# C0ldstudy/PointSecGuard

Hardware: AMD Instinct MI355X
Metric: attacked rooms/sec (4096 pts, 40 PGD iters) (higher is better)
Workload: dtype f32; 1 GPU; NB non-targeted PGD (eps=0.05, alpha=2/255, 40 iters) on PointNet++ SSG sem_seg, batch=8 rooms x 4096 pts x 9 ch per GPU (BASELINE configs[1]); steps_coalesced_per_launch_max=8, device_batch_rooms=64, launches_in_flight_per_gpu=3, weights=tests/golden/pn2_weights.npz (fitted fixture)

## Files before the change

pointsecguard_amd/csrc/psg_api.hip:

```cpp
#include <mutex>
#include <atomic>
#include <stdarg.h>
#include <stdlib.h>
#include <string.h>
#include <unordered_set>

#include "psg_common.h"

namespace {
thread_local char g_err[512] = "";
}

namespace psg {
struct EnvSwitch { const char *name; char kind; };
static const EnvSwitch kEnvSwitches[] = {
    {"PSG_TRACE_SYNC", 'd'},       {"PSG_GCN_KNN_STATS", 'd'},   {"PSG_KNN_XCD_ORDER", 'p'},  {"PSG_KNN_FINE_CUT_KK", 'p'},  {"PSG_KNN_SAMPLE2_KK", 'p'},  {"PSG_KNN_F32_SAMPLED_KK", 'p'},
    {"PSG_FP1_WAVE", 'p'},         {"PSG_RLA_NO_FUSE16", 'p'},   {"PSG_RLA_ATOMICS", 'p'},    {"PSG_RLA_NO_SPLIT", 'p'},
    {"PSG_RLA_NO_GRAPH", 'p'},     {"PSG_GEMM_SMALL_BELOW", 'p'}, {"PSG_GCN_KNN", 'p'},        {"PSG_GCN_KNN_BF_MAXD", 'p'},
    {"PSG_GCN_PQ_FUSION", 'p'},    {"PSG_GCN_NO_GRAPH", 'p'},    {"PSG_GCN_EDGE_BWD", 'p'},   {"PSG_BALL_QUERY", 'p'},
    {"PSG_PN2_SPLIT", 'p'},          {"PSG_RLA_NO_DIRECT", 'p'},   {"PSG_NU_NO_GRAPH", 'p'},      {"PSG_PN2_GRAPH", 'p'},
    {"PSG_PN2_FPSPLIT", 'p'},        {"PSG_FPS_CFG", 'p'},         {"PSG_PN2_L1T_COLOUR", 'p'},
    {"PSG_PN2_PGD_FUSE", 'p'},       {"PSG_PN2_POOLT_SPARSE", 'p'}, {"PSG_PN2_PW_SIZED", 'p'},
    {"PSG_PN2_BALL_TABLE", 'p'},     {"PSG_PN2_PACK", 'p'},          {"PSG_PN2_PACK_BWD", 'p'},
    {"PSG_PN2_POOLT_ORDER", 'p'},
#ifdef PSG_DIAG_BUILD
    {"PSG_DIAG", 'r'},
#endif
};

hipError_t copy_sync(void *dst, const void *src, size_t bytes, hipMemcpyKind kind)
{
    if (bytes == 0) return hipSuccess;
    hipStream_t st = nullptr;
    hipError_t e = hipStreamCreateWithFlags(&st, hipStreamNonBlocking);
    if (e != hipSuccess) return e;
    e = hipMemcpyAsync(dst, src, bytes, kind, st);
    if (e == hipSuccess) e = hipStreamSynchronize(st);
    (void)hipStreamDestroy(st);
    return e;
}

static std::atomic<uint64_t> g_generation{0};
uint64_t next_generation() { return ++g_generation; }

static std::atomic<long long> g_capture[4];
void capture_note(CaptureCounters *own, int tried, int failed, int replays, int eager)
{
    if (own) { own->tried += tried; own->failed += failed; own->replays += replays; own->eager += eager; }
    g_capture[0] += tried; g_capture[1] += failed; g_capture[2] += replays; g_capture[3] += eager;
}

bool GraphSlot::capture(hipStream_t st, const std::function<int()> &body)
{
    bool ok = false;
    if (hipStreamBeginCapture(st, hipStreamCaptureModeThreadLocal) == hipSuccess) {
        const int crc = body();
        hipGraph_t graph = nullptr;
        const hipError_t e = hipStreamEndCapture(st, &graph);
        ok = crc == PSG_OK && e == hipSuccess && graph && hipGraphInstantiate(&exec, graph, nullptr, nullptr, 0) == hipSuccess;
        if (!ok) exec = nullptr;
        if (graph) (void)hipGraphDestroy(graph);
    }
    (void)hipGetLastError();
    capture_failed = !ok;
    capture_note(&cap, 1, ok ? 0 : 1, 0, 0);
    return ok;
}

hipError_t GraphSlot::forget(hipStream_t st)
{
    if (exec) {
        const hipError_t e = hipStreamSynchronize(st);
        if (e != hipSuccess) return e;
        destroy();
    }
    capture_failed = false;
    return hipSuccess;
}

hipError_t GraphSlot::replay(hipStream_t st, int n)
{
    capture_note(&cap, 0, 0, n, 0);
    for (int i = 0; i < n; ++i) {
        const hipError_t e = hipGraphLaunch(exec, st);
        if (e != hipSuccess) return e;
    }
    return hipSuccess;
}

void GraphSlot::destroy()
{
    if (exec) (void)hipGraphExecDestroy(exec);
    exec = nullptr;
}

hipError_t memset_sync(void *dst, int value, size_t bytes)
{
    if (bytes == 0) return hipSuccess;
    hipStream_t st = nullptr;
    hipError_t e = hipStreamCreateWithFlags(&st, hipStreamNonBlocking);
    if (e != hipSuccess) return e;
    e = hipMemsetAsync(dst, value, bytes, st);
    if (e == hipSuccess) e = hipStreamSynchronize(st);
    (void)hipStreamDestroy(st);
    return e;
}

const char *env_str(const char *name)
{
    bool known = false;
    for (const EnvSwitch &e : kEnvSwitches) known = known || strcmp(e.name, name) == 0;
    if (!known) fprintf(stderr, "[psg] environment switch %s is read but not registered in psg_api.hip\n", name);
    return getenv(name);
}

int env_int(const char *name, int dflt)
{
    const char *v = env_str(name);
    return v ? atoi(v) : dflt;
}

bool trace_sync_enabled()
{
    static const bool on = env_int("PSG_TRACE_SYNC", 0) != 0;
    return on;
}

void trace_sync_point(const char *site)
{
    static unsigned long n = 0;
    const char *base = strrchr(site, '/');
    fprintf(stderr, "[psg trace] launch %lu at %s issued\n", ++n, base ? base + 1 : site);
    fflush(stderr);
    hipError_t e = hipDeviceSynchronize();
    fprintf(stderr, "[psg trace] launch %lu done (%s)\n", n, hipGetErrorString(e));
    fflush(stderr);
}

hipError_t allow_big_lds(const void *kern)
{
    static std::mutex mu;
    static std::unordered_set<const void *> done;
    std::lock_guard<std::mutex> lock(mu);
    if (done.count(kern)) return hipSuccess;
    hipFuncAttributes fa;
    hipError_t e = hipFuncGetAttributes(&fa, kern);
    if (e == hipSuccess) e = hipFuncSetAttribute(kern, hipFuncAttributeMaxDynamicSharedMemorySize, 160 * 1024 - (int)fa.sharedSizeBytes);
    if (e == hipSuccess) done.insert(kern);
    if (trace_sync_enabled()) fprintf(stderr, "[psg trace] LDS opt-in %zu (%s)\n", done.size(), hipGetErrorString(e));
    return e;
}

void set_error(const char *fmt, ...)
{
    va_list ap;
    va_start(ap, fmt);
    vsnprintf(g_err, sizeof(g_err), fmt, ap);
    va_end(ap);
}
}

extern "C" const char *psg_last_error(void) { return g_err; }

extern "C" int psg_env_switches(char *buf, int cap)
{
    PSG_REQUIRE(buf && cap > 0, "psg_env_switches: null / empty buffer");
    std::string out;
    int n = 0;
    for (const psg::EnvSwitch &e : psg::kEnvSwitches) {
        const char *v = getenv(e.name);
        if (!v) continue;
        out += std::string(e.name) + "=" + v + ":" + e.kind + ";";
        ++n;
    }
    PSG_REQUIRE((int)out.size() < cap, "psg_env_switches: buffer of %d bytes is too small (%d needed)", cap, (int)out.size() + 1);
    memcpy(buf, out.c_str(), out.size() + 1);
    return n;
}

extern "C" int psg_diag_build(void)
{
#ifdef PSG_DIAG_BUILD
    return 1;
#else
    return 0;
#endif
}

extern "C" int psg_capture_stats(long long *out4)
{
    PSG_REQUIRE(out4, "psg_capture_stats: null out pointer");
    for (int i = 0; i < 4; ++i) out4[i] = psg::g_capture[i].load();
    return PSG_OK;
}

extern "C" const char *psg_version(void) { return "libpsg 0.1 (gfx950, fp32 MFMA)"; }

extern "C" int psg_ctx_create(int device, psg_ctx **out)
{
    PSG_REQUIRE(out, "psg_ctx_create: null out pointer");
    int n = 0;
    PSG_CHECK_HIP(hipGetDeviceCount(&n));
    PSG_REQUIRE(device >= 0 && device < n, "psg_ctx_create: device %d not present (%d devices)", device, n);
    hipDeviceProp_t prop;
    PSG_CHECK_HIP(hipGetDeviceProperties(&prop, device));
    if (std::string(prop.gcnArchName).rfind("gfx950", 0) != 0) {
        psg::set_error("psg_ctx_create: device %d is %s; libpsg is built for gfx950 (MI355X) only", device,
                       prop.gcnArchName);
        return PSG_ERR_ARG;
    }
    PSG_CHECK_HIP(hipSetDevice(device));
    psg_ctx *c = new psg_ctx();
    c->device = device;
    c->num_cu = prop.multiProcessorCount;
    *out = c;
    return PSG_OK;
}

extern "C" int psg_ctx_destroy(psg_ctx *ctx)
{
    delete ctx;
    return PSG_OK;
}
```

pointsecguard_amd/csrc/psg_geometry.hip:

```cpp
#include "psg_common.h"
#include "psg_sqdist.cuh"

namespace {

using psg::sqdist;
using psg::sumsq3;

typedef float v2f __attribute__((ext_vector_type(2)));

template <int CTRL, int ROW_MASK>
__device__ __forceinline__ unsigned dpp_max_u32(unsigned v)
{
    unsigned o = (unsigned)__builtin_amdgcn_update_dpp(0, (int)v, CTRL, ROW_MASK, 0xF, false);
    return o > v ? o : v;
}
__device__ __forceinline__ unsigned row_max_u32(unsigned v)
{
    v = dpp_max_u32<0xB1, 0xF>(v);
    v = dpp_max_u32<0x4E, 0xF>(v);
    v = dpp_max_u32<0x141, 0xF>(v);
    v = dpp_max_u32<0x140, 0xF>(v);
    return v;
}
__device__ __forceinline__ unsigned wave_max_u32(unsigned v)
{
    v = row_max_u32(v);
    v = dpp_max_u32<0x142, 0xA>(v);
    v = dpp_max_u32<0x143, 0xC>(v);
    return (unsigned)__builtin_amdgcn_readlane((int)v, 63);
}
template <int N>
__device__ __forceinline__ unsigned max_of(const unsigned (&k)[N])
{
    constexpr int G = (N + 2) / 3;
    unsigned t[G];
#pragma unroll
    for (int g = 0; g < G; ++g) {
        unsigned a = k[3 * g];
        if (3 * g + 1 < N) a = max(a, k[3 * g + 1]);
        if (3 * g + 2 < N) a = max(a, k[3 * g + 2]);
        t[g] = a;
    }
    if constexpr (G == 1) return t[0];
    else return max_of<G>(t);
}

template <int NT, int PPT, bool LDSC>
__global__ __launch_bounds__(NT) void fps_kernel(const float *__restrict__ xyz, int n_clouds, int N, int S,
                                                 const int32_t *__restrict__ start, int32_t *__restrict__ out)
{
    constexpr int NW = NT / 64;
    extern __shared__ float smem[];
    float *s_xyz = smem;
    uint2 *s_part = (uint2 *)(smem + (LDSC ? NT * PPT * 3 : 0));

    const int p = blockIdx.x;
    const int tid = threadIdx.x, lane = tid & 63;
    const int wave = __builtin_amdgcn_readfirstlane(tid >> 6);
    const float *src = xyz + (size_t)(p % n_clouds) * N * 3;
    if (LDSC) {
        for (int i = tid; i < NT * PPT * 3; i += NT) s_xyz[i] = i < N * 3 ? src[i] : 0.0f;
        __syncthreads();
    }

    constexpr int PP = (PPT + 1) / 2;
    v2f px[PP], py[PP], pz[PP];
    unsigned dist[PPT];
#pragma unroll
    for (int q = 0; q < PP; ++q) {
        const int i = tid * PPT + 2 * q, i1 = (2 * q + 1 < PPT) ? i + 1 : i;
        if (LDSC) {
            px[q] = v2f{s_xyz[3 * i], s_xyz[3 * i1]};
            py[q] = v2f{s_xyz[3 * i + 1], s_xyz[3 * i1 + 1]};
            pz[q] = v2f{s_xyz[3 * i + 2], s_xyz[3 * i1 + 2]};
        } else {
            const bool in0 = i < N, in1 = i1 < N;
            px[q] = v2f{in0 ? src[3 * i] : 0.0f, in1 ? src[3 * i1] : 0.0f};
            py[q] = v2f{in0 ? src[3 * i + 1] : 0.0f, in1 ? src[3 * i1 + 1] : 0.0f};
            pz[q] = v2f{in0 ? src[3 * i + 2] : 0.0f, in1 ? src[3 * i1 + 2] : 0.0f};
        }
    }
#pragma unroll
    for (int j = 0; j < PPT; ++j) dist[j] = (tid * PPT + j) < N ? __float_as_uint(1e10f) : 0u;

    int far = start[p];
    int32_t *o = out + (size_t)p * S;
    for (int s = 0; s < S; ++s) {
        if (tid == 0) o[s] = far;
        float cx, cy, cz;
        if (LDSC) {
            cx = s_xyz[3 * far], cy = s_xyz[3 * far + 1], cz = s_xyz[3 * far + 2];
        } else {
            const float *c = src + 3 * (size_t)far;
            cx = c[0], cy = c[1], cz = c[2];
        }
        const v2f cx2 = {cx, cx}, cy2 = {cy, cy}, cz2 = {cz, cz};
#pragma unroll
        for (int q = 0; q < PP; ++q) {
            const v2f dx = px[q] - cx2, dy = py[q] - cy2, dz = pz[q] - cz2;
            const v2f d = ((dx * dx) + (dy * dy)) + (dz * dz);
            dist[2 * q] = min(dist[2 * q], __float_as_uint(d[0]));
            if (2 * q + 1 < PPT) dist[2 * q + 1] = min(dist[2 * q + 1], __float_as_uint(d[1]));
        }
        const unsigned best = max_of<PPT>(dist);
        const unsigned wmax = wave_max_u32(best);
        const unsigned long long hit = __ballot(best == wmax);
        const int src_lane = __builtin_ctzll(hit);
        int bq = PPT - 1;
#pragma unroll
        for (int j = PPT - 2; j >= 0; --j)
            if ((__ballot(dist[j] == wmax) >> src_lane) & 1ull) bq = j;
        int widx = (wave * 64 + src_lane) * PPT + bq;
        if (NW > 1) {
            uint2 *slot = s_part + (s & 1) * NW;
            if (lane == 0) slot[wave] = make_uint2(wmax, (unsigned)widx);
            __syncthreads();
            const uint2 part = slot[lane & (NW - 1)];
            const unsigned gmax = row_max_u32(part.x);
            const unsigned long long hw = __ballot(part.x == gmax) & ((1ull << NW) - 1ull);
            widx = __builtin_amdgcn_readlane((int)part.y, __builtin_ctzll(hw));
        }
        far = __builtin_amdgcn_readfirstlane(widx);
    }
}

__global__ void gather_rows_kernel(const float *__restrict__ pts, int n_clouds, int N, int C,
                                   const int32_t *__restrict__ idx, int S, float *__restrict__ out, int P)
{
    size_t total = (size_t)P * S * C;
    for (size_t t = (size_t)blockIdx.x * blockDim.x + threadIdx.x; t < total; t += (size_t)gridDim.x * blockDim.x) {
        int c = (int)(t % C);
        size_t r = t / C;
        int s = (int)(r % S);
        int p = (int)(r / S);
        out[t] = pts[((size_t)(p % n_clouds) * N + idx[(size_t)p * S + s]) * C + c];
    }
}

constexpr int BQ_THREADS = 1024;
constexpr int BQ_CPB = 128;
constexpr int BQ_UNROLL = 4;

__global__ __launch_bounds__(BQ_THREADS) void ball_query_kernel(const float *__restrict__ xyz, int n_clouds,
                                                                const float *__restrict__ new_xyz, int N, int S,
                                                                float r2, int K, int32_t *__restrict__ out)
{
    extern __shared__ float s_soa[];
    const int NP = (N + 255) & ~255;
    float *s_x = s_soa, *s_y = s_soa + NP, *s_z = s_soa + 2 * NP, *s_q = s_soa + 3 * NP;
    const int p = blockIdx.y;
    const float *src = xyz + (size_t)(p % n_clouds) * N * 3;
    for (int i = threadIdx.x; i < NP; i += BQ_THREADS) {
        float x = 0.f, y = 0.f, z = 0.f, q = INFINITY;
        if (i < N) { x = src[3 * i]; y = src[3 * i + 1]; z = src[3 * i + 2]; q = sumsq3(x, y, z); }
        s_x[i] = x; s_y[i] = y; s_z[i] = z; s_q[i] = q;
    }
    __syncthreads();
    const int lane = threadIdx.x & 63, wave = threadIdx.x >> 6;
    const unsigned long long lt_mask = (1ull << lane) - 1ull;
    const int c_end = min(S, (int)(blockIdx.x + 1) * BQ_CPB);
    for (int c = blockIdx.x * BQ_CPB + wave; c < c_end; c += BQ_THREADS / 64) {
        const float *cp = new_xyz + ((size_t)p * S + c) * 3;
        const float cx = cp[0], cy = cp[1], cz = cp[2];
        const float csq = sumsq3(cx, cy, cz);
        const v2f cx2 = {cx, cx}, cy2 = {cy, cy}, cz2 = {cz, cz}, cs2 = {csq, csq}, m2 = {-2.0f, -2.0f};
        int32_t *o = out + ((size_t)p * S + c) * K;
        int cnt = 0, first = N;
        for (int base = 0; base < N && cnt < K; base += 64 * BQ_UNROLL) {
            bool in[BQ_UNROLL];
#pragma unroll
            for (int u = 0; u < BQ_UNROLL; u += 2) {
                const int j = base + u * 64 + lane;
                const v2f qx = {s_x[j], s_x[j + 64]}, qy = {s_y[j], s_y[j + 64]}, qz = {s_z[j], s_z[j + 64]},
                          qs = {s_q[j], s_q[j + 64]};
                v2f dot = cx2 * qx;
                dot = __builtin_elementwise_fma(cy2, qy, dot);
                dot = __builtin_elementwise_fma(cz2, qz, dot);
                const v2f dd = ((m2 * dot) + cs2) + qs;
                in[u] = !(dd[0] > r2);
                in[u + 1] = !(dd[1] > r2);
            }
#pragma unroll
            for (int u = 0; u < BQ_UNROLL; ++u) {
                unsigned long long m = __ballot(in[u]);
                if (m) {
                    if (cnt == 0) first = base + u * 64 + __builtin_ctzll(m);
                    int pos = cnt + __popcll(m & lt_mask);
                    if (in[u] && pos < K) o[pos] = base + u * 64 + lane;
                    cnt += __popcll(m);
                }
            }
        }
        for (int pos = min(cnt, K) + lane; pos < K; pos += 64) o[pos] = first;
    }
}

constexpr int BQG_CELLS = 4096;
constexpr int BQG_CPB = 1024;

template <int CTRL, int ROW_MASK>
__device__ __forceinline__ unsigned bq_dpp0(unsigned v)
{
    return (unsigned)__builtin_amdgcn_update_dpp(0, (int)v, CTRL, ROW_MASK, 0xF, false);
}
__device__ __forceinline__ unsigned bq_wave_incl_scan(unsigned v)
{
    v += bq_dpp0<0x111, 0xF>(v);
    v += bq_dpp0<0x112, 0xF>(v);
    v += bq_dpp0<0x114, 0xF>(v);
    v += bq_dpp0<0x118, 0xF>(v);
    v += bq_dpp0<0x142, 0xA>(v);
    v += bq_dpp0<0x143, 0xC>(v);
    return v;
}

__global__ __launch_bounds__(BQ_THREADS) void ball_query_grid_kernel(const float *__restrict__ xyz, int n_clouds,
                                                                     const float *__restrict__ new_xyz, int N, int S,
                                                                     float r2, int K, int32_t *__restrict__ out)
{
    extern __shared__ float s_soa[];
    const int NP = (N + 255) & ~255;
    float *s_x = s_soa, *s_y = s_soa + NP, *s_z = s_soa + 2 * NP, *s_q = s_soa + 3 * NP;
    int *s_start = (int *)(s_soa + 4 * NP);
    int *s_cur = s_start + BQG_CELLS + 1;
    unsigned short *s_sorted = (unsigned short *)(s_cur + BQG_CELLS);
    __shared__ float s_red[BQ_THREADS / 64][6];
    __shared__ float s_box[8];
    __shared__ int s_dim[4];
    __shared__ int s_wsum[BQ_THREADS / 64];
    const int tid = threadIdx.x, lane = tid & 63, wave = tid >> 6;
    const int p = blockIdx.y;
    const float *src = xyz + (size_t)(p % n_clouds) * N * 3;
    float mn0 = INFINITY, mn1 = INFINITY, mn2 = INFINITY, mx0 = -INFINITY, mx1 = -INFINITY, mx2 = -INFINITY;
    for (int i = tid; i < NP; i += BQ_THREADS) {
        float x = 0.f, y = 0.f, z = 0.f, q = INFINITY;
        if (i < N) {
            x = src[3 * i]; y = src[3 * i + 1]; z = src[3 * i + 2]; q = sumsq3(x, y, z);
            mn0 = fminf(mn0, x); mn1 = fminf(mn1, y); mn2 = fminf(mn2, z);
            mx0 = fmaxf(mx0, x); mx1 = fmaxf(mx1, y); mx2 = fmaxf(mx2, z);
        }
        s_x[i] = x; s_y[i] = y; s_z[i] = z; s_q[i] = q;
    }
    for (int o = 32; o > 0; o >>= 1) {
        mn0 = fminf(mn0, __shfl_xor(mn0, o)); mn1 = fminf(mn1, __shfl_xor(mn1, o)); mn2 = fminf(mn2, __shfl_xor(mn2, o));
        mx0 = fmaxf(mx0, __shfl_xor(mx0, o)); mx1 = fmaxf(mx1, __shfl_xor(mx1, o)); mx2 = fmaxf(mx2, __shfl_xor(mx2, o));
    }
    if (lane == 0) { s_red[wave][0] = mn0; s_red[wave][1] = mn1; s_red[wave][2] = mn2; s_red[wave][3] = mx0; s_red[wave][4] = mx1; s_red[wave][5] = mx2; }
    __syncthreads();
    if (tid == 0) {
        float lo[3] = {INFINITY, INFINITY, INFINITY}, hi[3] = {-INFINITY, -INFINITY, -INFINITY};
        for (int w = 0; w < BQ_THREADS / 64; ++w)
            for (int a = 0; a < 3; ++a) { lo[a] = fminf(lo[a], s_red[w][a]); hi[a] = fmaxf(hi[a], s_red[w][3 + a]); }
        float maxabs = 0.0f;
        for (int a = 0; a < 3; ++a) maxabs = fmaxf(maxabs, fmaxf(fabsf(lo[a]), fabsf(hi[a])));
        maxabs += sqrtf(r2);
        float edge = 1.05f * sqrtf(r2 + 1e-5f * maxabs * maxabs);
        const bool finite = maxabs < 1e18f;
        int nx, ny, nz;
        for (;;) {
            if (!finite) { nx = ny = nz = 1; edge = 1.0f; break; }
            nx = (int)((hi[0] - lo[0]) / edge) + 1; ny = (int)((hi[1] - lo[1]) / edge) + 1; nz = (int)((hi[2] - lo[2]) / edge) + 1;
            if ((long long)nx * ny * nz <= BQG_CELLS) break;
            edge *= 1.25f;
        }
        s_box[0] = lo[0]; s_box[1] = lo[1]; s_box[2] = lo[2]; s_box[3] = 1.0f / edge;
        s_box[4] = hi[0]; s_box[5] = hi[1]; s_box[6] = hi[2]; s_box[7] = edge;
        s_dim[0] = nx; s_dim[1] = ny; s_dim[2] = nz; s_dim[3] = nx * ny * nz;
    }
    __syncthreads();
    const float bx = s_box[0], by = s_box[1], bz = s_box[2], inv = s_box[3];
    const float hx = s_box[4], hy = s_box[5], hz = s_box[6], edge1 = s_box[7];
    const int nx = s_dim[0], ny = s_dim[1], nz = s_dim[2], ncell = s_dim[3];
    auto cell1 = [&](float v, float b, int n) {
        if (n == 1) return 0;
        const int c = (int)((v - b) * inv);
        return c < 0 ? 0 : (c >= n ? n - 1 : c);
    };
    for (int c = tid; c <= ncell; c += BQ_THREADS) s_start[c] = 0;
    __syncthreads();
    for (int i = tid; i < N; i += BQ_THREADS)
        atomicAdd(&s_start[(cell1(s_z[i], bz, nz) * ny + cell1(s_y[i], by, ny)) * nx + cell1(s_x[i], bx, nx) + 1], 1);
    __syncthreads();
    {
        const int c0 = 1 + 4 * tid;
        int v[4], sum = 0;
#pragma unroll
        for (int u = 0; u < 4; ++u) { v[u] = c0 + u <= ncell ? s_start[c0 + u] : 0; sum += v[u]; v[u] = sum; }
        const int inc = (int)bq_wave_incl_scan((unsigned)sum);
        if (lane == 63) s_wsum[wave] = inc;
        __syncthreads();
        int base = inc - sum;
        for (int w = 0; w < wave; ++w) base += s_wsum[w];
#pragma unroll
        for (int u = 0; u < 4; ++u)
            if (c0 + u <= ncell) s_start[c0 + u] = base + v[u];
    }
    __syncthreads();
    for (int c = tid; c < ncell; c += BQ_THREADS) s_cur[c] = s_start[c];
    __syncthreads();
    for (int i = tid; i < N; i += BQ_THREADS) {
        const int cell = (cell1(s_z[i], bz, nz) * ny + cell1(s_y[i], by, ny)) * nx + cell1(s_x[i], bx, nx);
        s_sorted[atomicAdd(&s_cur[cell], 1)] = (unsigned short)i;
    }
    __syncthreads();
    const int words = NP >> 5;
    unsigned *bm = (unsigned *)s_cur + wave * words;
    const int c_end = min(S, (int)(blockIdx.x + 1) * BQG_CPB);
    for (int c = blockIdx.x * BQG_CPB + wave; c < c_end; c += BQ_THREADS / 64) {
        for (int w = lane; w < words; w += 64) bm[w] = 0u;
        const float *cp = new_xyz + ((size_t)p * S + c) * 3;
        const float cx = cp[0], cy = cp[1], cz = cp[2];
        const float csq = sumsq3(cx, cy, cz);
        const int ix = cell1(cx, bx, nx), iy = cell1(cy, by, ny), iz = cell1(cz, bz, nz);
        int start = 0, len = 0;
        const bool off_cloud = !(cx >= bx - edge1 && cx <= hx + edge1 && cy >= by - edge1 && cy <= hy + edge1 && cz >= bz - edge1 &&
                                 cz <= hz + edge1);
        if (off_cloud) {
            len = lane == 0 ? N : 0;
        } else if (lane < 9) {
            const int z = iz + lane / 3 - 1, y = iy + lane % 3 - 1;
            if (z >= 0 && z < nz && y >= 0 && y < ny) {
                const int x0 = ix > 0 ? ix - 1 : 0, x1 = ix + 1 < nx ? ix + 1 : nx - 1;
                const int lin = (z * ny + y) * nx + x0;
                start = s_start[lin];
                len = s_start[lin + (x1 - x0) + 1] - start;
            }
        }
        const int incl = (int)bq_wave_incl_scan((unsigned)len);
        const int T = __builtin_amdgcn_readlane(incl, 8);
        const int off = incl - len;
        __builtin_amdgcn_fence(__ATOMIC_SEQ_CST, "wavefront");
        __builtin_amdgcn_wave_barrier();
        for (int i0 = 0; i0 < T; i0 += 64) {
            const int i = i0 + lane;
            int pos = -1;
#pragma unroll
            for (int r = 0; r < 9; ++r) {
                const int o = __builtin_amdgcn_readlane(off, r), l = __builtin_amdgcn_readlane(len, r),
                          st = __builtin_amdgcn_readlane(start, r);
                pos = (i >= o && i < o + l) ? st + (i - o) : pos;
            }
            if (pos >= 0) {
                const int j = s_sorted[pos];
                const float dd = sqdist(cx, cy, cz, csq, s_x[j], s_y[j], s_z[j], s_q[j]);
                if (!(dd > r2)) atomicOr(&bm[j >> 5], 1u << (j & 31));
            }
        }
        __builtin_amdgcn_fence(__ATOMIC_SEQ_CST, "wavefront");
        __builtin_amdgcn_wave_barrier();
        int32_t *o = out + ((size_t)p * S + c) * K;
        int cnt = 0, first = N;
        for (int w0 = 0; w0 < words && cnt < K; w0 += 64) {
            unsigned word = w0 + lane < words ? bm[w0 + lane] : 0u;
            const int pc = __popc(word);
            const int inc = (int)bq_wave_incl_scan((unsigned)pc);
            const int tot = __builtin_amdgcn_readlane(inc, 63);
            if (tot == 0) continue;
            if (cnt == 0) {
                const int fl = __builtin_ctzll(__ballot(word != 0u));
                first = (w0 + fl) * 32 + __builtin_ctz((unsigned)__builtin_amdgcn_readlane((int)word, fl));
            }
            int rank = cnt + inc - pc;
            while (word && rank < K) {
                o[rank++] = (w0 + lane) * 32 + __builtin_ctz(word);
                word &= word - 1u;
            }
            cnt += tot;
        }
        for (int pos = min(cnt, K) + lane; pos < K; pos += 64) o[pos] = first;
        __builtin_amdgcn_wave_barrier();
    }
}
constexpr int NN_THREADS = 256;

__global__ __launch_bounds__(NN_THREADS) void three_nn_kernel(const float *__restrict__ xyz1, int n_clouds1,
                                                              const float *__restrict__ xyz2, int N, int S,
                                                              int32_t *__restrict__ idx, float *__restrict__ w)
{
    extern __shared__ float4 s_pair[];
    const int p = blockIdx.y;
    const float *c2 = xyz2 + (size_t)p * S * 3;
    const int S2 = (S + 1) >> 1;
    for (int i = threadIdx.x; i < S2; i += NN_THREADS) {
        const int a = 2 * i, b = 2 * i + 1;
        const float xa = c2[3 * a], ya = c2[3 * a + 1], za = c2[3 * a + 2];
        float xb = 0.f, yb = 0.f, zb = 0.f, sb = INFINITY;
        if (b < S) { xb = c2[3 * b]; yb = c2[3 * b + 1]; zb = c2[3 * b + 2]; sb = sumsq3(xb, yb, zb); }
        s_pair[2 * i] = make_float4(xa, xb, ya, yb);
        s_pair[2 * i + 1] = make_float4(za, zb, sumsq3(xa, ya, za), sb);
    }
    __syncthreads();
    const int i = blockIdx.x * NN_THREADS + threadIdx.x;
    if (i >= N) return;
    const float *fp = xyz1 + ((size_t)(p % n_clouds1) * N + i) * 3;
    const float fx = fp[0], fy = fp[1], fz = fp[2];
    const float fsq = sumsq3(fx, fy, fz);
    const v2f fx2 = {fx, fx}, fy2 = {fy, fy}, fz2 = {fz, fz}, fs2 = {fsq, fsq}, m2 = {-2.0f, -2.0f};
    float d0 = INFINITY, d1 = INFINITY, d2 = INFINITY;
    int i0 = 0, i1 = 0, i2 = 0;
    for (int jj = 0; jj < S2; ++jj) {
        const float4 q0 = s_pair[2 * jj], q1 = s_pair[2 * jj + 1];
        const v2f qx = {q0.x, q0.y}, qy = {q0.z, q0.w}, qz = {q1.x, q1.y}, qs = {q1.z, q1.w};
        v2f dot = fx2 * qx;
        dot = __builtin_elementwise_fma(fy2, qy, dot);
        dot = __builtin_elementwise_fma(fz2, qz, dot);
        const v2f dd = ((m2 * dot) + fs2) + qs;
#pragma unroll
        for (int u = 0; u < 2; ++u) {
            const float d = dd[u];
            const int j = 2 * jj + u;
            if (d < d2) {
                if (d < d1) {
                    d2 = d1; i2 = i1;
                    if (d < d0) { d1 = d0; i1 = i0; d0 = d; i0 = j; }
                    else { d1 = d; i1 = j; }
                } else { d2 = d; i2 = j; }
            }
        }
    }
    float r0 = __fdiv_rn(1.0f, __fadd_rn(d0, 1e-8f));
    float r1 = __fdiv_rn(1.0f, __fadd_rn(d1, 1e-8f));
    float r2 = __fdiv_rn(1.0f, __fadd_rn(d2, 1e-8f));
    float norm = __fadd_rn(__fadd_rn(r0, r1), r2);
    size_t o = ((size_t)p * N + i) * 3;
    idx[o] = i0; idx[o + 1] = i1; idx[o + 2] = i2;
    w[o] = __fdiv_rn(r0, norm); w[o + 1] = __fdiv_rn(r1, norm); w[o + 2] = __fdiv_rn(r2, norm);
}

__global__ void square_distance_kernel(const float *__restrict__ src, const float *__restrict__ dst, int N, int M,
                                       float *__restrict__ out)
{
    const int b = blockIdx.z;
    const int i = blockIdx.y;
    const float *s = src + ((size_t)b * N + i) * 3;
    const float sx = s[0], sy = s[1], sz = s[2];
    const float ssq = sumsq3(sx, sy, sz);
    for (int j = blockIdx.x * blockDim.x + threadIdx.x; j < M; j += gridDim.x * blockDim.x) {
        const float *d = dst + ((size_t)b * M + j) * 3;
        out[((size_t)b * N + i) * M + j] = sqdist(sx, sy, sz, ssq, d[0], d[1], d[2], sumsq3(d[0], d[1], d[2]));
    }
}

template <int NT, int PPT, bool LDSC = true>
int launch_fps(const float *xyz, int n_clouds, int P, int N, int S, const int32_t *start, int32_t *out,
               hipStream_t st)
{
    size_t lds = (LDSC ? (size_t)NT * PPT * 3 * 4 : 0) + 2 * (NT / 64) * 8;
    if (lds > 48 * 1024) PSG_CHECK_HIP(psg::allow_big_lds((const void *)fps_kernel<NT, PPT, LDSC>));
    hipLaunchKernelGGL((fps_kernel<NT, PPT, LDSC>), dim3(P), dim3(NT), lds, st, xyz, n_clouds, N, S, start, out);
    PSG_LAUNCH_CHECK();
    return PSG_OK;
}

}

extern "C" int psg_fps(psg_ctx *ctx, const float *xyz, int n_clouds, int P, int N, int S, const int32_t *start,
                       int32_t *out_idx, psg_stream stream)
{
    PSG_REQUIRE(ctx && xyz && start && out_idx, "psg_fps: null argument");
    PSG_REQUIRE(P > 0 && n_clouds > 0 && N > 0 && S > 0 && S <= N, "psg_fps: bad sizes P=%d N=%d S=%d", P, N, S);
    PSG_REQUIRE(N <= 8192, "psg_fps: N=%d exceeds the LDS-resident limit 8192", N);
    hipStream_t st = (hipStream_t)stream;
    if (N <= 64) return launch_fps<64, 1>(xyz, n_clouds, P, N, S, start, out_idx, st);
    if (N <= 256) return launch_fps<64, 4>(xyz, n_clouds, P, N, S, start, out_idx, st);
    if (N <= 1024) return launch_fps<256, 4>(xyz, n_clouds, P, N, S, start, out_idx, st);
    static const int cfg = psg::env_int("PSG_FPS_CFG", 0);
    if (N <= 4096 && cfg == 1) return launch_fps<1024, 4>(xyz, n_clouds, P, N, S, start, out_idx, st);
    if (N <= 4096 && cfg == 3) return launch_fps<256, 16>(xyz, n_clouds, P, N, S, start, out_idx, st);
    if (N <= 4096 && cfg == 5) return launch_fps<512, 8, false>(xyz, n_clouds, P, N, S, start, out_idx, st);
    if (N <= 4096 && (cfg == 4 || (cfg == 0 && P > 256))) return launch_fps<256, 16, false>(xyz, n_clouds, P, N, S, start, out_idx, st);
    if (N <= 4096) return launch_fps<512, 8>(xyz, n_clouds, P, N, S, start, out_idx, st);
    return launch_fps<1024, 8>(xyz, n_clouds, P, N, S, start, out_idx, st);
}

extern "C" int psg_square_distance(psg_ctx *ctx, const float *src, const float *dst, int B, int N, int M, float *out,
                                   psg_stream stream)
{
    PSG_REQUIRE(ctx && src && dst && out, "psg_square_distance: null argument");
    PSG_REQUIRE(B > 0 && N > 0 && M > 0 && N <= 65535 && B <= 65535, "psg_square_distance: bad sizes");
    hipLaunchKernelGGL(square_distance_kernel, dim3(std::min(64, psg::ceil_div(M, 256)), N, B), dim3(256), 0,
                       (hipStream_t)stream, src, dst, N, M, out);
    PSG_LAUNCH_CHECK();
    return PSG_OK;
}

extern "C" int psg_gather_points(psg_ctx *ctx, const float *points, int n_clouds, int P, int N, int C,
                                 const int32_t *idx, int S, float *out, psg_stream stream)
{
    PSG_REQUIRE(ctx && points && idx && out, "psg_gather_points: null argument");
    PSG_REQUIRE(P > 0 && n_clouds > 0 && N > 0 && C > 0 && S > 0, "psg_gather_points: bad sizes");
    size_t total = (size_t)P * S * C;
    int blocks = (int)std::min<size_t>((total + 255) / 256, 4096);
    hipLaunchKernelGGL(gather_rows_kernel, dim3(blocks), dim3(256), 0, (hipStream_t)stream, points, n_clouds, N, C,
                       idx, S, out, P);
    PSG_LAUNCH_CHECK();
    return PSG_OK;
}

extern "C" int psg_ball_query(psg_ctx *ctx, const float *xyz, int n_clouds, const float *new_xyz, int P, int N,
                              int S, float r2, int K, int32_t *out_idx, psg_stream stream)
{
    PSG_REQUIRE(ctx && xyz && new_xyz && out_idx, "psg_ball_query: null argument");
    PSG_REQUIRE(P > 0 && n_clouds > 0 && N > 0 && S > 0 && K > 0, "psg_ball_query: bad sizes");
    PSG_REQUIRE(N <= 8192, "psg_ball_query: N=%d exceeds the LDS-resident limit 8192", N);
    static const bool scan_only = []() { const char *v = psg::env_str("PSG_BALL_QUERY"); return v && std::string(v) == "scan"; }();
    const size_t soa = (size_t)((N + 255) & ~255) * 4 * sizeof(float);
    if (!scan_only && N >= 2048 && N <= 4096 && r2 > 0.0f && r2 < 1e30f) {
        const size_t lds = soa + (size_t)(2 * BQG_CELLS + 1) * 4 + (size_t)((N + 255) & ~255) * 2;
        if (lds > 48 * 1024) PSG_CHECK_HIP(psg::allow_big_lds((const void *)ball_query_grid_kernel));
        hipLaunchKernelGGL(ball_query_grid_kernel, dim3(psg::ceil_div(S, BQG_CPB), P), dim3(BQ_THREADS), lds, (hipStream_t)stream, xyz,
                           n_clouds, new_xyz, N, S, r2, K, out_idx);
        PSG_LAUNCH_CHECK();
        return PSG_OK;
    }
    if (soa > 48 * 1024) PSG_CHECK_HIP(psg::allow_big_lds((const void *)ball_query_kernel));
    hipLaunchKernelGGL(ball_query_kernel, dim3(psg::ceil_div(S, BQ_CPB), P), dim3(BQ_THREADS), soa,
                       (hipStream_t)stream, xyz, n_clouds, new_xyz, N, S, r2, K, out_idx);
    PSG_LAUNCH_CHECK();
    return PSG_OK;
}

extern "C" int psg_three_nn(psg_ctx *ctx, const float *xyz1, int n_clouds1, const float *xyz2, int P, int N, int S,
                            int32_t *out_idx, float *out_w, psg_stream stream)
{
    PSG_REQUIRE(ctx && xyz1 && xyz2 && out_idx && out_w, "psg_three_nn: null argument");
    PSG_REQUIRE(P > 0 && n_clouds1 > 0 && N > 0 && S >= 3, "psg_three_nn: bad sizes (need S >= 3)");
    PSG_REQUIRE(S <= 8192, "psg_three_nn: S=%d exceeds the LDS-resident limit 8192", S);
    size_t lds = (size_t)2 * ((S + 1) / 2) * sizeof(float4);
    if (lds > 48 * 1024) PSG_CHECK_HIP(psg::allow_big_lds((const void *)three_nn_kernel));
    hipLaunchKernelGGL(three_nn_kernel, dim3(psg::ceil_div(N, NN_THREADS), P), dim3(NN_THREADS), lds,
                       (hipStream_t)stream, xyz1, n_clouds1, xyz2, N, S, out_idx, out_w);
    PSG_LAUNCH_CHECK();
    return PSG_OK;
}
```

Before: 1024 rooms/s.

## Add uniform-grid three-NN kernel for large feature-propagation interpolation

Adds a three_nn grid kernel. It bins the source points into an LDS-resident uniform grid via counting sort, sorts the queries by cell, and walks the neighbouring cells with an exact termination bound. Queries with non-finite inputs or out-of-box positions fall back to a full scan. The goal is to replace the O(N·S) brute-force scan for large clouds (N≥2048, S between 512 and 1024, P≥320), selectable through the PSG_THREE_NN switch. The cost is extra setup passes, atomics and barriers per block, plus tie-break and rounding-slack logic that must reproduce the brute-force neighbour choice.

Measured after the change: 1041 rooms/s (median of 6 runs). 1.02x the previous value.

```diff
diff --git a/pointsecguard_amd/csrc/psg_api.hip b/pointsecguard_amd/csrc/psg_api.hip
--- a/pointsecguard_amd/csrc/psg_api.hip
+++ b/pointsecguard_amd/csrc/psg_api.hip
@@ -22,7 +22,7 @@
     {"PSG_PN2_FPSPLIT", 'p'},        {"PSG_FPS_CFG", 'p'},         {"PSG_PN2_L1T_COLOUR", 'p'},
     {"PSG_PN2_PGD_FUSE", 'p'},       {"PSG_PN2_POOLT_SPARSE", 'p'}, {"PSG_PN2_PW_SIZED", 'p'},
     {"PSG_PN2_BALL_TABLE", 'p'},     {"PSG_PN2_PACK", 'p'},          {"PSG_PN2_PACK_BWD", 'p'},
-    {"PSG_PN2_POOLT_ORDER", 'p'},
+    {"PSG_PN2_POOLT_ORDER", 'p'},    {"PSG_THREE_NN", 'p'},
 #ifdef PSG_DIAG_BUILD
     {"PSG_DIAG", 'r'},
 #endif
diff --git a/pointsecguard_amd/csrc/psg_geometry.hip b/pointsecguard_amd/csrc/psg_geometry.hip
--- a/pointsecguard_amd/csrc/psg_geometry.hip
+++ b/pointsecguard_amd/csrc/psg_geometry.hip
@@ -427,6 +427,267 @@
     w[o] = __fdiv_rn(r0, norm); w[o + 1] = __fdiv_rn(r1, norm); w[o + 2] = __fdiv_rn(r2, norm);
 }
 
+constexpr int NNG_THREADS = 512;
+constexpr int NNG_CELLS = 2 * NNG_THREADS;
+constexpr int NNG_MAX_S = 1024;
+constexpr float NNG_PPC = 2.0f;
+constexpr float NNG_ERR = 1e-5f;
+constexpr float NNG_SLACK = 4e-6f;
+
+__device__ __forceinline__ int nn_uni(int v) { return __builtin_amdgcn_readfirstlane(v); }
+__device__ __forceinline__ float nn_uni(float v) { return __int_as_float(__builtin_amdgcn_readfirstlane(__float_as_int(v))); }
+__device__ __forceinline__ bool nn_before(float d, int j, float bd, int bj) { return d < bd || (d == bd && j < bj); }
+
+__global__ __launch_bounds__(NNG_THREADS) void three_nn_grid_kernel(const float *__restrict__ xyz1, int n_clouds1,
+                                                                    const float *__restrict__ xyz2, int N, int S, int qpb,
+                                                                    int32_t *__restrict__ idx, float *__restrict__ w)
+{
+    extern __shared__ float4 s_pt[];
+    float4 *s_sp = s_pt + S;
+    int *s_start = (int *)(s_sp + S);
+    int *s_cur = s_start + NNG_CELLS + 1;
+    unsigned short *s_sj = (unsigned short *)(s_cur + NNG_CELLS + 1);
+    unsigned short *s_qs = s_sj + S;
+    __shared__ float s_red[NNG_THREADS / 64][6];
+    __shared__ float s_box[8];
+    __shared__ int s_dim[4];
+    __shared__ int s_wsum[NNG_THREADS / 64];
+    __shared__ int s_bad;
+    const int tid = threadIdx.x, lane = tid & 63, wave = tid >> 6;
+    const int p = blockIdx.y;
+    const float *c2 = xyz2 + (size_t)p * S * 3;
+    if (tid == 0) s_bad = 0;
+    __syncthreads();
+    float mn0 = INFINITY, mn1 = INFINITY, mn2 = INFINITY, mx0 = -INFINITY, mx1 = -INFINITY, mx2 = -INFINITY;
+    bool bad = false;
+    for (int i = tid; i < S; i += NNG_THREADS) {
+        const float x = c2[3 * i], y = c2[3 * i + 1], z = c2[3 * i + 2];
+        s_pt[i] = make_float4(x, y, z, sumsq3(x, y, z));
+        mn0 = fminf(mn0, x); mn1 = fminf(mn1, y); mn2 = fminf(mn2, z);
+        mx0 = fmaxf(mx0, x); mx1 = fmaxf(mx1, y); mx2 = fmaxf(mx2, z);
+        bad = bad || !(fmaxf(fmaxf(fabsf(x), fabsf(y)), fabsf(z)) < 1e18f) || x != x || y != y || z != z;
+    }
+    for (int o = 32; o > 0; o >>= 1) {
+        mn0 = fminf(mn0, __shfl_xor(mn0, o)); mn1 = fminf(mn1, __shfl_xor(mn1, o)); mn2 = fminf(mn2, __shfl_xor(mn2, o));
+        mx0 = fmaxf(mx0, __shfl_xor(mx0, o)); mx1 = fmaxf(mx1, __shfl_xor(mx1, o)); mx2 = fmaxf(mx2, __shfl_xor(mx2, o));
+    }
+    if (lane == 0) { s_red[wave][0] = mn0; s_red[wave][1] = mn1; s_red[wave][2] = mn2; s_red[wave][3] = mx0; s_red[wave][4] = mx1; s_red[wave][5] = mx2; }
+    if (bad) s_bad = 1;
+    __syncthreads();
+    const bool scan_all = nn_uni(s_bad) != 0;
+    float bx = 0.f, by = 0.f, bz = 0.f, inv = 1.f, hx = 0.f, hy = 0.f, hz = 0.f, edge = 1.f;
+    int nx = 1, ny = 1, nz = 1;
+    if (!scan_all) {
+        if (tid == 0) {
+            float lo[3] = {INFINITY, INFINITY, INFINITY}, hi[3] = {-INFINITY, -INFINITY, -INFINITY};
+            for (int wv = 0; wv < NNG_THREADS / 64; ++wv) {
+#pragma unroll
+                for (int a = 0; a < 3; ++a) { lo[a] = fminf(lo[a], s_red[wv][a]); hi[a] = fmaxf(hi[a], s_red[wv][3 + a]); }
+            }
+            const float ex = hi[0] - lo[0], ey = hi[1] - lo[1], ez = hi[2] - lo[2];
+            const float emax = fmaxf(ex, fmaxf(ey, ez));
+            float e = 1.0f;
+            int dx = 1, dy = 1, dz = 1;
+            if (emax > 0.0f) {
+                const float fl = emax * (1.0f / 64.0f);
+                e = cbrtf(fmaxf(ex, fl) * fmaxf(ey, fl) * fmaxf(ez, fl) * (NNG_PPC / (float)S));
+                for (;;) {
+                    dx = (int)(ex / e) + 1; dy = (int)(ey / e) + 1; dz = (int)(ez / e) + 1;
+                    if ((long long)dx * dy * dz <= NNG_CELLS) break;
+                    e *= 1.25f;
+                }
+            }
+            s_box[0] = lo[0]; s_box[1] = lo[1]; s_box[2] = lo[2]; s_box[3] = 1.0f / e;
+            s_box[4] = hi[0]; s_box[5] = hi[1]; s_box[6] = hi[2]; s_box[7] = e;
+            s_dim[0] = dx; s_dim[1] = dy; s_dim[2] = dz; s_dim[3] = dx * dy * dz;
+        }
+        __syncthreads();
+        bx = nn_uni(s_box[0]); by = nn_uni(s_box[1]); bz = nn_uni(s_box[2]); inv = nn_uni(s_box[3]);
+        hx = nn_uni(s_box[4]); hy = nn_uni(s_box[5]); hz = nn_uni(s_box[6]); edge = nn_uni(s_box[7]);
+        nx = nn_uni(s_dim[0]); ny = nn_uni(s_dim[1]); nz = nn_uni(s_dim[2]);
+    }
+    const int ncell = nx * ny * nz;
+    auto cell1 = [&](float v, float b, int n) { return (int)fminf(fmaxf((v - b) * inv, 0.0f), (float)(n - 1)); };
+    auto scan_counts = [&](int *a) {
+        const int c0 = 1 + 2 * tid;
+        const int v0 = c0 <= ncell ? a[c0] : 0, v1 = c0 + 1 <= ncell ? a[c0 + 1] : 0;
+        const int inc = (int)bq_wave_incl_scan((unsigned)(v0 + v1));
+        if (lane == 63) s_wsum[wave] = inc;
+        __syncthreads();
+        int base = inc;
+        for (int wv = 0; wv < wave; ++wv) base += s_wsum[wv];
+        if (c0 <= ncell) a[c0] = base - v1;
+        if (c0 + 1 <= ncell) a[c0 + 1] = base;
+        __syncthreads();
+    };
+    const float *f1 = xyz1 + (size_t)(p % n_clouds1) * N * 3;
+    const int q_begin = blockIdx.x * qpb, nq = min(N, q_begin + qpb) - q_begin;
+    auto cell_of = [&](float x, float y, float z) { return (cell1(z, bz, nz) * ny + cell1(y, by, ny)) * nx + cell1(x, bx, nx); };
+    if (!scan_all) {
+        for (int c = tid; c <= ncell; c += NNG_THREADS) s_start[c] = 0;
+        __syncthreads();
+        for (int i = tid; i < S; i += NNG_THREADS) {
+            const float4 q = s_pt[i];
+            atomicAdd(&s_start[cell_of(q.x, q.y, q.z) + 1], 1);
+        }
+        __syncthreads();
+        scan_counts(s_start);
+        for (int c = tid; c <= ncell; c += NNG_THREADS) s_cur[c] = c < ncell ? s_start[c] : 0;
+        __syncthreads();
+        for (int i = tid; i < S; i += NNG_THREADS) {
+            const float4 q = s_pt[i];
+            const int pos = atomicAdd(&s_cur[cell_of(q.x, q.y, q.z)], 1);
+            s_sp[pos] = q;
+            s_sj[pos] = (unsigned short)i;
+        }
+        __syncthreads();
+        for (int c = tid; c <= ncell; c += NNG_THREADS) s_cur[c] = 0;
+        __syncthreads();
+        for (int t = tid; t < nq; t += NNG_THREADS) {
+            const float *fp = f1 + (size_t)(q_begin + t) * 3;
+            atomicAdd(&s_cur[cell_of(fp[0], fp[1], fp[2]) + 1], 1);
+        }
+        __syncthreads();
+        scan_counts(s_cur);
+        for (int t = tid; t < nq; t += NNG_THREADS) {
+            const float *fp = f1 + (size_t)(q_begin + t) * 3;
+            s_qs[atomicAdd(&s_cur[cell_of(fp[0], fp[1], fp[2])], 1)] = (unsigned short)t;
+        }
+    }
+    __syncthreads();
+    const float span = (float)max(nx, max(ny, nz)) * edge;
+    const float box_abs = fmaxf(fmaxf(fmaxf(fabsf(bx), fabsf(by)), fabsf(bz)), fmaxf(fmaxf(fabsf(hx), fabsf(hy)), fabsf(hz)));
+    for (int g = wave; g * 64 < nq; g += NNG_THREADS / 64) {
+        const int t = g * 64 + lane;
+        const bool live = t < nq;
+        const int i = q_begin + (live ? (scan_all ? t : (int)s_qs[t]) : 0);
+        const float *fp = f1 + (size_t)i * 3;
+        const float fx = fp[0], fy = fp[1], fz = fp[2];
+        const float fsq = sumsq3(fx, fy, fz);
+        float d0 = INFINITY, d1 = INFINITY, d2 = INFINITY;
+        int i0 = 0, i1 = 0, i2 = 0;
+        auto take = [&](float d, int j) {
+            if (nn_before(d, j, d2, i2)) {
+                const bool b1 = nn_before(d, j, d1, i1), b0 = nn_before(d, j, d0, i0);
+                d2 = b1 ? d1 : d; i2 = b1 ? i1 : j;
+                d1 = b0 ? d0 : (b1 ? d : d1); i1 = b0 ? i0 : (b1 ? j : i1);
+                d0 = b0 ? d : d0; i0 = b0 ? j : i0;
+            }
+        };
+        auto cand = [&](int pos) {
+            const float4 q = s_sp[pos];
+            take(sqdist(fx, fy, fz, fsq, q.x, q.y, q.z, q.w), (int)s_sj[pos]);
+        };
+        const bool far = scan_all || !(fx >= bx - span && fx <= hx + span && fy >= by - span && fy <= hy + span &&
+                                       fz >= bz - span && fz <= hz + span);
+        const bool walks = live && !far;
+        const int cx = cell1(fx, bx, nx), cy = cell1(fy, by, ny), cz = cell1(fz, bz, nz);
+        const float maxabs = fmaxf(box_abs, fmaxf(fmaxf(fabsf(fx), fabsf(fy)), fabsf(fz)));
+        const float err = NNG_ERR * (maxabs * maxabs), slack = NNG_SLACK * maxabs;
+        auto done = [&](int k) {
+            float L = INFINITY;
+            if (cx - k > 0) L = fminf(L, fx - (bx + (float)(cx - k) * edge));
+            if (cx + k < nx - 1) L = fminf(L, (bx + (float)(cx + k + 1) * edge) - fx);
+            if (cy - k > 0) L = fminf(L, fy - (by + (float)(cy - k) * edge));
+            if (cy + k < ny - 1) L = fminf(L, (by + (float)(cy + k + 1) * edge) - fy);
+            if (cz - k > 0) L = fminf(L, fz - (bz + (float)(cz - k) * edge));
+            if (cz + k < nz - 1) L = fminf(L, (bz + (float)(cz + k + 1) * edge) - fz);
+            if (L == INFINITY) return true;
+            const float Ls = L - slack;
+            return Ls > 0.0f && Ls * Ls - err > d2;
+        };
+        bool alone = false;
+        if (__any(walks)) {
+            int x0 = walks ? cx : nx, x1 = walks ? cx : -1, y0 = walks ? cy : ny, y1 = walks ? cy : -1, z0 = walks ? cz : nz, z1 = walks ? cz : -1;
+            for (int o = 32; o > 0; o >>= 1) {
+                x0 = min(x0, __shfl_xor(x0, o)); y0 = min(y0, __shfl_xor(y0, o)); z0 = min(z0, __shfl_xor(z0, o));
+                x1 = max(x1, __shfl_xor(x1, o)); y1 = max(y1, __shfl_xor(y1, o)); z1 = max(z1, __shfl_xor(z1, o));
+            }
+            x0 = max(__builtin_amdgcn_readfirstlane(x0) - 1, 0); x1 = min(__builtin_amdgcn_readfirstlane(x1) + 1, nx - 1);
+            y0 = max(__builtin_amdgcn_readfirstlane(y0) - 1, 0); y1 = min(__builtin_amdgcn_readfirstlane(y1) + 1, ny - 1);
+            z0 = max(__builtin_amdgcn_readfirstlane(z0) - 1, 0); z1 = min(__builtin_amdgcn_readfirstlane(z1) + 1, nz - 1);
+            const bool all_x = x0 == 0 && x1 == nx - 1;
+            const int ys = all_x ? y1 - y0 + 1 : 1;
+            const int zs = all_x && ys == ny ? z1 - z0 + 1 : 1;
+            if (walks) {
+                for (int z = z0; z <= z1; z += zs)
+                    for (int y = y0; y <= y1; y += ys) {
+                        const int end = nn_uni(s_start[((z + zs - 1) * ny + (y + ys - 1)) * nx + x1 + 1]);
+                        for (int pos = nn_uni(s_start[(z * ny + y) * nx + x0]); pos < end; pos += 4) {
+                            float d[4];
+#pragma unroll
+                            for (int u = 0; u < 4; ++u) {
+                                const float4 q = s_sp[min(pos + u, S - 1)];
+                                d[u] = sqdist(fx, fy, fz, fsq, q.x, q.y, q.z, q.w);
+                            }
+#pragma unroll
+                            for (int u = 0; u < 4; ++u)
+                                if (pos + u < end && d[u] <= d2) take(d[u], (int)s_sj[pos + u]);
+                        }
+                    }
+            }
+            alone = walks && !done(1);
+        }
+        if (alone) {
+            d0 = d1 = d2 = INFINITY; i0 = i1 = i2 = 0;
+            {
+                const int x0 = max(cx - 1, 0), xn = min(cx + 1, nx - 1) - x0 + 1;
+                int r = 0, pos = 0, end = 0;
+                for (;;) {
+                    while (pos >= end && r < 9) {
+                        const int rz = (r * 11) >> 5;
+                        const int z = cz + rz - 1, y = cy + (r - 3 * rz) - 1;
+                        if (z >= 0 && z < nz && y >= 0 && y < ny) {
+                            const int lin = (z * ny + y) * nx + x0;
+                            pos = s_start[lin]; end = s_start[lin + xn];
+                        }
+                        ++r;
+                    }
+                    if (pos >= end) break;
+                    cand(pos++);
+                }
+            }
+            for (int k = 1; !done(k); ++k) {
+                const int kk = k + 1;
+                for (int z = max(cz - kk, 0); z <= min(cz + kk, nz - 1); ++z)
+                    for (int y = max(cy - kk, 0); y <= min(cy + kk, ny - 1); ++y) {
+                        const int row = (z * ny + y) * nx;
+                        const bool rim = z - cz == kk || cz - z == kk || y - cy == kk || cy - y == kk;
+                        if (rim) {
+                            const int end = s_start[row + min(cx + kk, nx - 1) + 1];
+                            for (int pos = s_start[row + max(cx - kk, 0)]; pos < end; ++pos) cand(pos);
+                        } else {
+                            if (cx - kk >= 0) { const int end = s_start[row + cx - kk + 1]; for (int pos = s_start[row + cx - kk]; pos < end; ++pos) cand(pos); }
+                            if (cx + kk < nx) { const int end = s_start[row + cx + kk + 1]; for (int pos = s_start[row + cx + kk]; pos < end; ++pos) cand(pos); }
+                        }
+                    }
+            }
+        }
+        if (live && far) {
+            for (int j = 0; j < S; ++j) {
+                const float4 q = s_pt[j];
+                const float d = sqdist(fx, fy, fz, fsq, q.x, q.y, q.z, q.w);
+                if (d < d2) {
+                    if (d < d1) {
+                        d2 = d1; i2 = i1;
+                        if (d < d0) { d1 = d0; i1 = i0; d0 = d; i0 = j; }
+                        else { d1 = d; i1 = j; }
+                    } else { d2 = d; i2 = j; }
+                }
+            }
+        }
+        if (live) {
+            float r0 = __fdiv_rn(1.0f, __fadd_rn(d0, 1e-8f));
+            float r1 = __fdiv_rn(1.0f, __fadd_rn(d1, 1e-8f));
+            float r2 = __fdiv_rn(1.0f, __fadd_rn(d2, 1e-8f));
+            float norm = __fadd_rn(__fadd_rn(r0, r1), r2);
+            size_t o = ((size_t)p * N + i) * 3;
+            idx[o] = i0; idx[o + 1] = i1; idx[o + 2] = i2;
+            w[o] = __fdiv_rn(r0, norm); w[o + 1] = __fdiv_rn(r1, norm); w[o + 2] = __fdiv_rn(r2, norm);
+        }
+    }
+}
+
 __global__ void square_distance_kernel(const float *__restrict__ src, const float *__restrict__ dst, int N, int M,
                                        float *__restrict__ out)
 {
@@ -526,6 +787,19 @@
     PSG_REQUIRE(ctx && xyz1 && xyz2 && out_idx && out_w, "psg_three_nn: null argument");
     PSG_REQUIRE(P > 0 && n_clouds1 > 0 && N > 0 && S >= 3, "psg_three_nn: bad sizes (need S >= 3)");
     PSG_REQUIRE(S <= 8192, "psg_three_nn: S=%d exceeds the LDS-resident limit 8192", S);
+    static const int mode = []() {
+        const char *v = psg::env_str("PSG_THREE_NN");
+        return !v ? 0 : std::string(v) == "scan" ? 1 : std::string(v) == "grid" ? 2 : 0;
+    }();
+    if (S <= NNG_MAX_S && (mode == 2 || (mode == 0 && N >= 2048 && S >= 512 && P >= 320))) {
+        const int qpb = (size_t)P * psg::ceil_div(N, 1024) > 2048 ? 4096 : 1024;
+        const size_t glds = (size_t)S * (2 * sizeof(float4) + 2) + (size_t)(2 * NNG_CELLS + 2) * 4 + (size_t)qpb * 2;
+        if (glds + 1024 > 48 * 1024) PSG_CHECK_HIP(psg::allow_big_lds((const void *)three_nn_grid_kernel));
+        hipLaunchKernelGGL(three_nn_grid_kernel, dim3(psg::ceil_div(N, qpb), P), dim3(NNG_THREADS), glds, (hipStream_t)stream,
+                           xyz1, n_clouds1, xyz2, N, S, qpb, out_idx, out_w);
+        PSG_LAUNCH_CHECK();
+        return PSG_OK;
+    }
     size_t lds = (size_t)2 * ((S + 1) / 2) * sizeof(float4);
     if (lds > 48 * 1024) PSG_CHECK_HIP(psg::allow_big_lds((const void *)three_nn_kernel));
     hipLaunchKernelGGL(three_nn_kernel, dim3(psg::ceil_div(N, NN_THREADS), P), dim3(NN_THREADS), lds,
```
